# kerry-he/fsae-mpc

Hardware: AMD Instinct MI355X
Metric: QP solves/sec (batched LTV-MPC, N=40 nx=5 nu=2 fp64) (higher is better)
Workload: dtype f64

## Files before the change

### fsae-mpc_amd/csrc/qp_solver.hip

```cpp
#include <hip/hip_runtime.h>
#include <math.h>
#include <stdint.h>
#include <stdlib.h>
#include <stdio.h>
#include "qp_solver.h"

typedef double v4d __attribute__((ext_vector_type(4)));
typedef double v2d __attribute__((ext_vector_type(2)));

#define DEVINL __device__ __forceinline__
#ifndef QP_SOLVE_REFINE_STEPS
#define QP_SOLVE_REFINE_STEPS 1
#endif
#ifndef QP_FULL_BARRIERS
#define WAVE_SYNC() do { __builtin_amdgcn_fence(__ATOMIC_SEQ_CST, "wavefront"); __builtin_amdgcn_wave_barrier(); } while (0)
#else
#define WAVE_SYNC() __syncthreads()
#endif

namespace {

DEVINL double rl(double v, int src) {
  int lo = __builtin_amdgcn_readlane(__double2loint(v), src);
  int hi = __builtin_amdgcn_readlane(__double2hiint(v), src);
// ... 47 lines not shown
  __host__ __device__ static constexpr int idx(int I, int J) { return I * T - (I * (I - 1)) / 2 + (J - I); }
};

#if !defined(QP_TU) || QP_TU == 0
#define QP_MAIN_TU 1
#else
#define QP_MAIN_TU 0
#endif

#if QP_MAIN_TU
__global__ __launch_bounds__(1024) void qp_prep_kernel(QpParams P) {
  const int b = blockIdx.x, tid = threadIdx.x, w = tid >> 6, lane = tid & 63, c = lane & 15, q = lane >> 4;
  const int NTH = blockDim.x, NW = NTH >> 6;
  const QpDims& d = P.d;
  const int n = d.n, nu = d.nu, m = d.m, T = d.T, Kq = d.Kq, J = d.J, JB = d.JB, np = d.np, nc = d.nc, nb = d.nb;
  const double* H = P.H + (P.shared_HA ? 0 : (size_t)b * nu * nu);
  const double* A = P.A + (P.shared_HA ? 0 : (size_t)b * m * nu);
  const double* g = P.g + (size_t)b * nu;
  auto U = [&](int i) { return qp_user_index(d, i); };
  auto Hat = [&](int i, int j) -> double { const int ui = U(i), uj = U(j); return (ui >= 0 && uj >= 0) ? H[(size_t)uj * nu + ui] : ((i == j && i < n) ? 1.0 : 0.0); };
  auto Aat = [&](int r, int j) -> double { const int uj = U(j); return uj >= 0 ? A[(size_t)uj * m + r] : 0.0; };
  double* ws = P.ws + (size_t)b * d.ws_per_qp;
  double* Aw = ws + d.off_Aw;
  double* Hw = ws + d.off_Hw;
  double* gw = ws + d.off_gw;
  double* Es = ws + d.off_E;
  double* Fs = ws + d.off_F;
  double* Ab = ws + d.off_Ab;
  double* Hb = ws + d.off_Hb;
  int* perm_g = reinterpret_cast<int*>(ws + d.off_meta);
  int* tcs_g = perm_g + (size_t)(J > 0 ? J : 1) * 64;
  int* aoff_g = tcs_g + d.ntr;
  int* tend_g = aoff_g + d.ntr + 1;
  const int ntr = d.ntr;
  double* Lr = ws + d.off_rows + 0 * (size_t)d.rowlen;
  double* Ur = ws + d.off_rows + 1 * (size_t)d.rowlen;
  extern __shared__ double lds[];
  double* Esh = lds;
  double* red = lds + np;
  double* tile = red + 16;
  const int TW = d.prep_tw;
  int* cls_sh = reinterpret_cast<int*>(tile + TW * (4 * Kq + 1));
  int* perm_sh = cls_sh + 4 * Kq;
  int* cnt_sh = perm_sh + 16 * ntr;
  int* tcs_sh = cnt_sh + 16;
  int* aoff_sh = tcs_sh + ntr;
  int* chc_sh = aoff_sh + ntr + 1;
  double* Fr_sh = reinterpret_cast<double*>((reinterpret_cast<uintptr_t>(chc_sh + ((m + 63) >> 6) * 16) + 7) & ~(uintptr_t)7);

  for (int j = tid; j < np; j += NTH) {
    double e = 1.0;
    if (j < n) {
      double hjj = Hat(j, j);
      if (hjj > 1e-12) e = 1.0 / sqrt(hjj);
      else e = -1.0;
    } else e = 0.0;
    Esh[j] = e;
  }
  __syncthreads();
  for (int j = 0; j < n; ++j) {
    if (Esh[j] < 0) {
      double cm = 0;
      for (int r = tid; r < m; r += NTH) cm = fmax(cm, fabs(Aat(r, j)));
      cm = wave_max(cm);
      if (lane == 0) red[w] = cm;
      __syncthreads();
      if (tid == 0) { double mx = 0.0; for (int i = 0; i < NW; ++i) mx = fmax(mx, red[i]); Esh[j] = mx > 1e-12 ? 1.0 / mx : 1.0; }
      __syncthreads();
    }
  }
  int bad = 0;
  for (int j = tid; j < np; j += NTH) { const int uj = j < n ? U(j) : -1; const double gj = uj >= 0 ? g[uj] : 0.0; Es[j] = Esh[j]; gw[j] = gj * Esh[j]; bad |= !(fabs(gj) < INFINITY); }

  __syncthreads();
  const int ncols = nc < n ? nc : n;
  const int nchunk = (m + 63) >> 6;
  for (int i = tid; i < nchunk * 16; i += NTH) chc_sh[i] = 0;
  if (tid < 16) cnt_sh[tid] = 0;
  __syncthreads();
  for (int r0 = 0; r0 < m; r0 += NTH) {
    const int r = r0 + tid;
    int e = 0;
    double rm = 0.0;
    if (r < m) {
      for (int col0 = 0; col0 < n; col0 += 8) {
        double av[8];
#pragma unroll
        for (int u = 0; u < 8; ++u) av[u] = col0 + u < n ? Aat(r, col0 + u) : 0.0;
#pragma unroll
        for (int u = 0; u < 8; ++u) {
          const int col = col0 + u;
          const double a = fabs(av[u]);
          if (col < n) { rm = fmax(rm, a * Esh[col]); if (a != 0.0 && col < ncols) e = col >> 4; }
        }
      }
      cls_sh[r] = e;
      Fr_sh[r] = rm > 1e-12 ? 1.0 / rm : 1.0;
    }
    for (int cl = 0; cl < T; ++cl) {
      const unsigned long long mk = __ballot(r < m && e == cl);
      if (lane == 0 && r0 + 64 * w < m) chc_sh[((r0 >> 6) + w) * 16 + cl] = __popcll(mk);
    }
  }
  __syncthreads();
  if (tid < T) {
    int tot = 0;
    for (int ch = 0; ch < nchunk; ++ch) tot += chc_sh[ch * 16 + tid];
    cnt_sh[tid] = tot;
  }
  __syncthreads();
  if (tid < T) {
    int start = 0;
    for (int cl = 0; cl < tid; ++cl) start += cnt_sh[cl];
    for (int ch = 0; ch < nchunk; ++ch) { const int cn = chc_sh[ch * 16 + tid]; chc_sh[ch * 16 + tid] = start; start += cn; }
  }
  for (int p = tid; p < 16 * ntr; p += NTH) perm_sh[p] = -1;
  __syncthreads();
  for (int r0 = 0; r0 < m; r0 += NTH) {
    const int r = r0 + tid;
    const int e = r < m ? cls_sh[r] : -1;
    for (int cl = 0; cl < T; ++cl) {
      const unsigned long long mk = __ballot(e == cl);
      if (e == cl) perm_sh[chc_sh[((r0 >> 6) + w) * 16 + cl] + __popcll(mk & ((1ull << lane) - 1ull))] = r;
    }
  }
  __syncthreads();
  for (int tr = tid; tr < ntr; tr += NTH) {
    int tc = 1;
    for (int p = 16 * tr; p < 16 * tr + 16; ++p) { const int r = perm_sh[p]; if (r >= 0) tc = max(tc, cls_sh[r] + 1); }
    tcs_sh[tr] = tc;
  }
  __syncthreads();
  if (tid == 0) {
    int run = 0;
    for (int tr = 0; tr < ntr; ++tr) { aoff_sh[tr] = run; run += 2 * tcs_sh[tr]; }
    aoff_sh[ntr] = run;
    for (int C = 0; C <= T; ++C) { int cn = 0; for (int tr = 0; tr < ntr; ++tr) cn += (tcs_sh[tr] <= C); tend_g[C] = cn; }
  }
  __syncthreads();
  for (int tr = tid; tr <= ntr; tr += NTH) { aoff_g[tr] = aoff_sh[tr]; if (tr < ntr) tcs_g[tr] = tcs_sh[tr]; }

  int nexcl = 0;
  for (int js = w; js < J; js += NW) {
    const int s = 16 * js + c, pp = 4 * s + q;
    const int r = (s < 4 * ntr) ? perm_sh[pp] : -1;
    const bool valid = r >= 0;
    const double f = valid ? Fr_sh[r] : 0.0;
    Fs[js * 64 + lane] = f;
    perm_g[js * 64 + lane] = r;
    for (int bb = 0; bb < 4; ++bb)
    { const double v = (valid && bb < nb) ? Aat(r, nc + bb) * Esh[nc + bb] * f : 0.0; bad |= !(fabs(v) < INFINITY); Ab[(size_t)bb * J * 64 + js * 64 + lane] = v; }
    double l = -INFINITY, u = INFINITY;
    if (valid) {
      double lr = P.lbA[(size_t)b * m + r], ur = P.ubA[(size_t)b * m + r];
      bad |= (lr != lr) || (ur != ur);
      nexcl += (lr > 0.0) || (ur < 0.0);
      l = lr > -P.inf_bound ? lr * f : -INFINITY;
      u = ur < P.inf_bound ? ur * f : INFINITY;
    }
    Lr[js * 64 + lane] = l;
    Ur[js * 64 + lane] = u;
  }
  for (int jb = w; jb < JB; jb += NW) {
    const int i = jb * 64 + lane;
    double l = -INFINITY, u = INFINITY;
    const int ui = i < n ? U(i) : -1;
    if (ui >= 0) {
      double lr = P.lb[(size_t)b * nu + ui], ur = P.ub[(size_t)b * nu + ui];
      bad |= (lr != lr) || (ur != ur);
      nexcl += (lr > 0.0) || (ur < 0.0);
      l = lr > -P.inf_bound ? lr / Esh[i] : -INFINITY;
      u = ur < P.inf_bound ? ur / Esh[i] : INFINITY;
    }
    Lr[(J + jb) * 64 + lane] = l;
    Ur[(J + jb) * 64 + lane] = u;
  }
  __syncthreads();

  const int R4 = 4 * Kq, mp1 = R4 + 1;
  for (int t = 0; t < T; ++t)
    for (int c0 = 0; c0 < 16; c0 += TW) {
      for (int e = tid; e < TW * R4; e += NTH) {
        const int cc = e / R4, r = e - cc * R4;
        const int col = 16 * t + c0 + cc;
        double v = 0.0;
        if (col < nc && col < n && r < m) v = Aat(r, col) * Esh[col];
        bad |= !(fabs(v) < INFINITY);
        tile[cc * mp1 + r] = v;
      }
      __syncthreads();
      for (int s = w; s < 4 * ntr; s += NW) {
        const int tr = s >> 2, tc = tcs_sh[tr];
        if (t < tc && c >= c0 && c < c0 + TW) {
          const int r = perm_sh[4 * s + q];
          const double v = r >= 0 ? tile[(c - c0) * mp1 + r] * Fr_sh[r] : 0.0;
          Aw[((size_t)aoff_sh[tr] + ((s >> 1) & 1) * tc + t) * 128 + lane * 2 + (s & 1)] = v;
        }
      }
      __syncthreads();
    }

  for (int idx = w; idx < T * T * 4; idx += NW) {
    const int p = idx & 3, IJ = idx >> 2, I = IJ / T, Jt = IJ - I * T;
    const int row = 16 * I + q + 4 * p, col = 16 * Jt + c;
    double v = 0.0;
    if (row < nc && col < nc && row < n && col < n) v = Hat(col, row) * Esh[row] * Esh[col];
    bad |= !(fabs(v) < INFINITY);
    Hw[(size_t)idx * 64 + lane] = v;
  }
  for (int e = tid; e < 4 * np; e += NTH) {
    const int bb = e / np, i = e - bb * np;
    const double v = (bb < nb && i < n) ? Hat(i, nc + bb) * Esh[nc + bb] * Esh[i] : 0.0;
    bad |= !(fabs(v) < INFINITY);
    Hb[e] = v;
  }
  bad = __syncthreads_or(bad);
  if (tid == 0) ws[d.off_bad] = bad ? 1.0 : 0.0;
  if (P.score) {
    __shared__ int score_sh;
    if (tid == 0) score_sh = 0;
    __syncthreads();
    if (nexcl) atomicAdd(&score_sh, nexcl);
    __syncthreads();
    if (tid == 0) P.score[b] = P.score_in ? P.score_in[b] : score_sh;
  }
}

__global__ __launch_bounds__(1024) void qp_order_kernel(const int* __restrict__ score, int* __restrict__ order, int batch) {
  constexpr int NBIN = 1024, NWV = 8;
  __shared__ int cnt[NWV][NBIN], scan[NBIN];
  const int tid = threadIdx.x, w = tid >> 6, lane = tid & 63;
  for (int e = tid; e < NWV * NBIN; e += 1024) (&cnt[0][0])[e] = 0;
  __syncthreads();
  const int per = ((batch + NWV - 1) / NWV + 63) & ~63;
  const int lo = w * per, hi = min(batch, lo + per);
  auto bin = [&](int i) { return NBIN - 1 - min(max(score[i], 0), NBIN - 1); };
  auto group = [&](int k, bool on, int& rank, int& size) {
    unsigned long long same = __builtin_amdgcn_ballot_w64(on);
#pragma unroll
    for (int bit = 0; bit < 10; ++bit) {
      const bool one = (k >> bit) & 1;
      const unsigned long long v = __builtin_amdgcn_ballot_w64(one);
      same &= one ? v : ~v;
    }
    rank = __popcll(same & ((1ull << lane) - 1ull)); size = __popcll(same);
  };
  if (w < NWV)
    for (int i0 = lo; i0 < hi; i0 += 512) {
      int kv[8];
#pragma unroll
      for (int r = 0; r < 8; ++r) { const int i = i0 + 64 * r + lane; kv[r] = i < hi ? bin(i) : -1; }
#pragma unroll
      for (int r = 0; r < 8; ++r) {
        const bool on = kv[r] >= 0; const int k = on ? kv[r] : 0;
        int rank, size; group(k, on, rank, size);
        if (on && rank == 0) cnt[w][k] += size;
      }
    }
  __syncthreads();
  int v = 0;
  for (int ww = 0; ww < NWV; ++ww) v += cnt[ww][tid];
  scan[tid] = v;
  __syncthreads();
  for (int o = 1; o < NBIN; o <<= 1) {
    const int a = tid >= o ? scan[tid - o] : 0;
    __syncthreads();
    scan[tid] += a;
    __syncthreads();
  }
  int run = scan[tid] - v;
  for (int ww = 0; ww < NWV; ++ww) { const int c = cnt[ww][tid]; cnt[ww][tid] = run; run += c; }
  __syncthreads();
  if (w < NWV)
    for (int i0 = lo; i0 < hi; i0 += 512) {
      int kv[8];
#pragma unroll
      for (int r = 0; r < 8; ++r) { const int i = i0 + 64 * r + lane; kv[r] = i < hi ? bin(i) : -1; }
#pragma unroll
      for (int r = 0; r < 8; ++r) {
        const bool on = kv[r] >= 0; const int k = on ? kv[r] : 0;
        int rank, size; group(k, on, rank, size);
        int base = on ? cnt[w][k] : 0;
        if (on) order[base + rank] = i0 + 64 * r + lane;
        if (on && rank == 0) cnt[w][k] = base + size;
      }
    }
}

#endif

struct Ctx {
  int n, m, T, Kq, J, JB, JT, np, ld, lane, c, q, nc, nb, ntr;
  const int* perm; const int* tcs; const int* aoff; const int* tend;
  const double* Aw; const double* Hw; const double* Ab; const double* Hb;
  double* rows;
  double* ring;
  double* cof;
  int rowlen;
  double* Ms;
  double* vec;
};
enum VecArr { V_X = 0, V_G, V_HX, V_R1, V_R2, V_P1, V_P2, V_P3, V_DX, V_E, V_NARR };

DEVINL double* rowp(const Ctx& k, int arr) { return k.rows + (size_t)arr * k.rowlen; }
DEVINL double* vecp(const Ctx& k, int arr) { return k.vec + arr * k.np; }

DEVINL bool row_valid(const Ctx& k, int js) {
  if (js < k.J) { const int s = 16 * js + k.c; return s < k.Kq && 4 * s + k.q < k.m; }
  return (js - k.J) * 64 + k.lane < k.n;
}

template <int T> DEVINL void hx_tiles(const Ctx& k, const double* X, double* HX) {
  double hx[T], hn[T][4], hc[T][4];
#pragma unroll
  for (int t = 0; t < T; ++t) hx[t] = 0.0;
#pragma unroll
  for (int Jt = 0; Jt < T; ++Jt)
#pragma unroll
    for (int p = 0; p < 4; ++p) hn[Jt][p] = k.Hw[((size_t)Jt * 4 + p) * 64 + k.lane];
#pragma unroll 1
  for (int I = 0; I < T; ++I) {
#pragma unroll
    for (int Jt = 0; Jt < T; ++Jt)
#pragma unroll
      for (int p = 0; p < 4; ++p) hc[Jt][p] = hn[Jt][p];
    if (I + 1 < T) {
#pragma unroll
      for (int Jt = 0; Jt < T; ++Jt)
#pragma unroll
        for (int p = 0; p < 4; ++p) hn[Jt][p] = k.Hw[((size_t)((I + 1) * T + Jt) * 4 + p) * 64 + k.lane];
    }
    double xk[4];
#pragma unroll
    for (int p = 0; p < 4; ++p) xk[p] = X[16 * I + k.q + 4 * p];
#pragma unroll
    for (int Jt = 0; Jt < T; ++Jt)
#pragma unroll
      for (int p = 0; p < 4; ++p) hx[Jt] = fma(hc[Jt][p], xk[p], hx[Jt]);
  }
#pragma unroll
  for (int t = 0; t < T; ++t) {
    double v = q_sum(hx[t]);
    if (k.q == 0) HX[16 * t + k.c] = v;
  }
}
template <int T> DEVINL void acc_init(const Ctx& k, v4d* acc) {
#pragma unroll
  for (int I = 0; I < T; ++I)
#pragma unroll
    for (int Jt = I; Jt < T; ++Jt) {
      const double* hp = k.Hw + ((size_t)(I * T + Jt) * 4) * 64 + k.lane;
      v4d h;
#pragma unroll
      for (int p = 0; p < 4; ++p) h[p] = hp[p * 64];
      acc[Tri<T>::idx(I, Jt)] = h;
    }
}

template <int T> DEVINL void hx_from_acc(const Ctx& k, const v4d* acc, const double* XV, double* HX) {
  double xr[T][4], xc[T], sc[T], sr[T][4];
#pragma unroll
  for (int I = 0; I < T; ++I) {
    xc[I] = XV[16 * I + k.c]; sc[I] = 0.0;
#pragma unroll
    for (int p = 0; p < 4; ++p) { xr[I][p] = XV[16 * I + k.q + 4 * p]; sr[I][p] = 0.0; }
  }
#pragma unroll
  for (int I = 0; I < T; ++I)
#pragma unroll
    for (int J = I; J < T; ++J) {
      const v4d& h = acc[Tri<T>::idx(I, J)];
#pragma unroll
      for (int p = 0; p < 4; ++p) {
        sc[J] = fma(h[p], xr[I][p], sc[J]);
        if (J > I) sr[I][p] = fma(h[p], xc[J], sr[I][p]);
      }
    }
  WAVE_SYNC();
#pragma unroll
  for (int J = 0; J < T; ++J) { const double v = q_sum(sc[J]); if (k.q == 0) HX[16 * J + k.c] = v; }
  WAVE_SYNC();
#pragma unroll
  for (int I = 0; I < T - 1; ++I)
#pragma unroll
    for (int p = 0; p < 4; ++p) { const double v = grp16_sum(sr[I][p]); if (k.c == 0) HX[16 * I + k.q + 4 * p] += v; }
}

template <int C> struct IC { static constexpr int value = C; };

#ifdef QP_DRAIN_STREAM
template <int T> struct StreamCfg {
  static constexpr int R = 3 * T;
};
template <int T> struct Stream {
  static constexpr int R = StreamCfg<T>::R;
  const char* gnext;
  int half;
  DEVINL void issue(const Ctx& k, int slot) {
    __builtin_amdgcn_global_load_lds((const __attribute__((address_space(1))) void*)(gnext + k.lane * 16),
                                     (__attribute__((address_space(3))) void*)(k.ring + slot * 128), 16, 0, 0);
    gnext += 1024;
  }
  DEVINL void start(const Ctx& k, int c0) {
    gnext = reinterpret_cast<const char*>(k.Aw); half = 0;
#pragma unroll
    for (int t = 0; t < T; ++t) if (t < c0) issue(k, t);
  }
  template <int C> DEVINL void next_pair(const Ctx& k, v2d* b, int cn) {
    asm volatile("s_waitcnt vmcnt(0)" ::: "memory");
    const int other = (half ^ 1) * T;
#pragma unroll
    for (int t = 0; t < T; ++t) if (t < cn) issue(k, other + t);
    asm volatile("" ::: "memory");
#pragma unroll
    for (int t = 0; t < C; ++t) b[t] = *reinterpret_cast<const v2d*>(k.ring + (half * T + t) * 128 + k.lane * 2);
    half ^= 1;
  }
  DEVINL void drain() { asm volatile("s_waitcnt vmcnt(0)" ::: "memory"); }
};
#else
template <int T> struct StreamCfg {
  static constexpr int D = 2 * T;
  static constexpr int R = D + T;
};
template <int T> struct Stream {
  static constexpr int D = StreamCfg<T>::D, R = StreamCfg<T>::R;
  const char* gnext; int slot_i, slot_e;
  DEVINL void issue(const Ctx& k) {
    __builtin_amdgcn_global_load_lds((const __attribute__((address_space(1))) void*)(gnext + k.lane * 16),
                                     (__attribute__((address_space(3))) void*)(k.ring + slot_i * 128), 16, 0, 0);
    gnext += 1024;
    slot_i = slot_i + 1 == R ? 0 : slot_i + 1;
  }
  DEVINL void start(const Ctx& k, int) {
    gnext = reinterpret_cast<const char*>(k.Aw); slot_i = 0; slot_e = 0;
#pragma unroll
    for (int j = 0; j < D; ++j) issue(k);
  }
  template <int C> DEVINL void next_pair(const Ctx& k, v2d* b, int) {
#pragma unroll
    for (int t = 0; t < C; ++t) issue(k);
    asm volatile("s_waitcnt vmcnt(%0)" :: "n"(D) : "memory");
#pragma unroll
    for (int t = 0; t < C; ++t) {
      int sl = slot_e + t; if (sl >= R) sl -= R;
      b[t] = *reinterpret_cast<const v2d*>(k.ring + sl * 128 + k.lane * 2);
    }
    slot_e += C; if (slot_e >= R) slot_e -= R;
  }
  DEVINL void drain() { asm volatile("s_waitcnt vmcnt(0)" ::: "memory"); }
};
#endif

template <int NA> struct CoefStage {
  double reg[NA > 0 ? NA : 1];
  DEVINL void load(const Ctx& k, const double* const* arr, int js) {
    const int jc = js < k.J ? js : k.J - 1;
#pragma unroll
    for (int a = 0; a < NA; ++a) reg[a] = arr[a][jc * 64 + k.lane];
  }
  DEVINL void commit(const Ctx& k) {
#pragma unroll
    for (int a = 0; a < NA; ++a) k.cof[a * 64 + k.lane] = reg[a];
  }
  DEVINL void read_pair(const Ctx& k, int s, v2d* out) const {
#pragma unroll
    for (int a = 0; a < NA; ++a) out[a] = *reinterpret_cast<const v2d*>(k.cof + a * 64 + k.q * 16 + (s & 15));
  }
};

template <int T, int NB> DEVINL void pass_syrk(const Ctx& k, v4d* acc, double* P1, double* P2, double* P3, double* MB) {
  constexpr int NBB = NB > 0 ? NB : 1;
  constexpr int NA = 4 + NB;
  const int JS = k.J * 64;
  const double* arr[NA];
  arr[0] = rowp(k, R_D); arr[1] = rowp(k, R_W1); arr[2] = rowp(k, R_W2); arr[3] = rowp(k, R_W3);
#pragma unroll
  for (int e = 0; e < NB; ++e) arr[4 + e] = k.Ab + (size_t)e * JS;
  double p1[T], p2[T], p3[T];
  double pb[NBB][T], sbb[NBB][NBB], pwb[3][NBB];
#pragma unroll
  for (int t = 0; t < T; ++t) { p1[t] = 0; p2[t] = 0; p3[t] = 0; }
#pragma unroll
  for (int e = 0; e < NBB; ++e) {
#pragma unroll
    for (int t = 0; t < T; ++t) pb[e][t] = 0;
#pragma unroll
    for (int f = 0; f < NBB; ++f) sbb[e][f] = 0;
    pwb[0][e] = pwb[1][e] = pwb[2][e] = 0;
  }
  Stream<T> st;
  CoefStage<NA> cs;
  int tr = 0;
  if (k.ntr > 0) { st.start(k, k.tcs[0]); cs.load(k, arr, 0); }
  auto phase = [&](auto Cc) __attribute__((always_inline)) {
    constexpr int C = decltype(Cc)::value;
    const int tr_end = k.tend[C];
    for (; tr < tr_end; ++tr) {
      if ((tr & 3) == 0) { cs.commit(k); cs.load(k, arr, (tr >> 2) + 1); }
#pragma unroll
      for (int u = 0; u < 2; ++u) {
        v2d b[C], cf[NA];
        st.template next_pair<C>(k, b, u == 0 ? C : (tr + 1 < tr_end ? C : (tr + 1 < k.ntr ? k.tcs[tr + 1] : 0)));
        cs.read_pair(k, 4 * tr + 2 * u, cf);
        asm volatile("" ::: "memory");
#pragma unroll
        for (int h = 0; h < 2; ++h) {
          double a[C], ab[NBB];
          const double dd = cf[0][h], w1 = cf[1][h], w2 = cf[2][h], w3 = cf[3][h];
#pragma unroll
          for (int e = 0; e < NB; ++e) ab[e] = cf[4 + e][h];
#pragma unroll
          for (int t = 0; t < C; ++t) a[t] = dd * b[t][h];
#pragma unroll
          for (int I = 0; I < C; ++I)
#pragma unroll
            for (int Jt = I; Jt < C; ++Jt)
              acc[Tri<T>::idx(I, Jt)] = __builtin_amdgcn_mfma_f64_16x16x4f64(a[I], b[Jt][h], acc[Tri<T>::idx(I, Jt)], 0, 0, 0);
#pragma unroll
          for (int t = 0; t < C; ++t) {
            p1[t] = fma(w1, b[t][h], p1[t]); p2[t] = fma(w2, b[t][h], p2[t]); p3[t] = fma(w3, b[t][h], p3[t]);
          }
#pragma unroll
          for (int e = 0; e < NB; ++e) {
            const double dab = dd * ab[e];
#pragma unroll
            for (int t = 0; t < C; ++t) pb[e][t] = fma(dab, b[t][h], pb[e][t]);
#pragma unroll
            for (int f = e; f < NB; ++f) sbb[e][f] = fma(dab, ab[f], sbb[e][f]);
            pwb[0][e] = fma(w1, ab[e], pwb[0][e]); pwb[1][e] = fma(w2, ab[e], pwb[1][e]); pwb[2][e] = fma(w3, ab[e], pwb[2][e]);
          }
        }
      }
    }
  };
  if constexpr (T >= 1) phase(IC<1>{});
  if constexpr (T >= 2) phase(IC<2>{});
  if constexpr (T >= 3) phase(IC<3>{});
  if constexpr (T >= 4) phase(IC<4>{});
  if constexpr (T >= 5) phase(IC<5>{});
  if constexpr (T >= 6) phase(IC<6>{});
  if constexpr (T >= 7) phase(IC<7>{});
  if constexpr (T >= 8) phase(IC<8>{});
  if (k.ntr > 0) st.drain();
#pragma unroll
  for (int t = 0; t < T; ++t) {
    double v1 = q_sum(p1[t]), v2 = q_sum(p2[t]), v3 = q_sum(p3[t]);
    if (k.q == 0) { P1[16 * t + k.c] = v1; P2[16 * t + k.c] = v2; P3[16 * t + k.c] = v3; }
  }
#pragma unroll
  for (int e = 0; e < NB; ++e) {
#pragma unroll
    for (int t = 0; t < T; ++t) { const double vb = q_sum(pb[e][t]); if (k.q == 0) MB[e * k.np + 16 * t + k.c] = vb; }
    const double v1 = q_sum(pwb[0][e]), v2 = q_sum(pwb[1][e]), v3 = q_sum(pwb[2][e]);
    if (k.lane == 0) { P1[k.nc + e] = v1; P2[k.nc + e] = v2; P3[k.nc + e] = v3; }
#pragma unroll
    for (int f = 0; f < NB; ++f) {
      const double sv = q_sum(f >= e ? sbb[e][f] : sbb[f][e]);
      if (k.lane == 0) MB[e * k.np + k.nc + f] = sv;
    }
  }
}

template <int T, int NB, int NVEC, int FUSE> DEVINL void pass_Av(const Ctx& k, const double* const* vin, double* const* rout, double* Pcor, double* Pcor2 = nullptr, const double* const* cfarr = nullptr) {
  constexpr int NBB = NB > 0 ? NB : 1;
  constexpr int NC = FUSE == 1 ? 6 : (FUSE >= 2 ? 3 : 0);
  constexpr int NA = NC + NB;
  const int JS = k.J * 64;
  const double* arr[NA > 0 ? NA : 1];
  if (FUSE == 1) { arr[0] = rowp(k, R_RPL); arr[1] = rowp(k, R_CB1); arr[2] = rowp(k, R_CC1); arr[3] = rowp(k, R_RPU); arr[4] = rowp(k, R_CB2); arr[5] = rowp(k, R_CC2); }
  if (FUSE >= 2) { arr[0] = cfarr ? cfarr[0] : rowp(k, R_CB1); arr[1] = cfarr ? cfarr[1] : rowp(k, R_RPL); arr[2] = cfarr ? cfarr[2] : rowp(k, R_CC1); }
#pragma unroll
  for (int f = 0; f < NB; ++f) arr[NC + f] = k.Ab + (size_t)f * JS;
  double v[NVEC][T], vb[NVEC][NBB], pc[T], pcb[NBB], pd[FUSE >= 2 ? T : 1], pdb[NBB];
#pragma unroll
  for (int e = 0; e < NVEC; ++e) {
#pragma unroll
    for (int t = 0; t < T; ++t) v[e][t] = vin[e][16 * t + k.c];
#pragma unroll
    for (int f = 0; f < NB; ++f) vb[e][f] = vin[e][k.nc + f];
  }
#pragma unroll
  for (int t = 0; t < T; ++t) pc[t] = 0.0;
#pragma unroll
  for (int f = 0; f < NBB; ++f) { pcb[f] = 0.0; pdb[f] = 0.0; }
#pragma unroll
  for (int t = 0; t < (FUSE >= 2 ? T : 1); ++t) pd[t] = 0.0;
  double keep[NVEC + 1];
#pragma unroll
  for (int e = 0; e < NVEC + 1; ++e) keep[e] = 0.0;
  Stream<T> st;
  CoefStage<NA> cs;
  int tr = 0;
  if (k.ntr > 0) { st.start(k, k.tcs[0]); if (NA > 0) cs.load(k, arr, 0); }
  auto phase = [&](auto Cc) __attribute__((always_inline)) {
    constexpr int C = decltype(Cc)::value;
    const int tr_end = k.tend[C];
    for (; tr < tr_end; ++tr) {
      if (NA > 0 && (tr & 3) == 0) { cs.commit(k); cs.load(k, arr, (tr >> 2) + 1); }
#pragma unroll
      for (int u = 0; u < 2; ++u) {
        v2d b[C], cf[NA > 0 ? NA : 1];
        st.template next_pair<C>(k, b, u == 0 ? C : (tr + 1 < tr_end ? C : (tr + 1 < k.ntr ? k.tcs[tr + 1] : 0)));
        if (NA > 0) cs.read_pair(k, 4 * tr + 2 * u, cf);
        asm volatile("" ::: "memory");
#pragma unroll
        for (int h = 0; h < 2; ++h) {
          const int s = 4 * tr + 2 * u + h;
          const int cc = s & 15;
#pragma unroll
          for (int e = 0; e < NVEC; ++e) {
            double dsum = 0.0;
#pragma unroll
            for (int t = 0; t < C; ++t) dsum = fma(b[t][h], v[e][t], dsum);
            dsum = grp16_sum(dsum);
#pragma unroll
            for (int f = 0; f < NB; ++f) dsum = fma(cf[NC + f][h], vb[e][f], dsum);
            if (k.c == cc) keep[e] = dsum;
            if (FUSE >= 2 && e == 0) {
              const double pen = cf[0][h] * (dsum - cf[1][h]);
              const double ynew = cf[2][h] - pen;
              if (k.c == cc) keep[NVEC] = ynew;
#pragma unroll
              for (int t = 0; t < C; ++t) { pc[t] = fma(ynew, b[t][h], pc[t]); pd[t] = fma(pen, b[t][h], pd[t]); }
#pragma unroll
              for (int f = 0; f < NB; ++f) { pcb[f] = fma(ynew, cf[NC + f][h], pcb[f]); pdb[f] = fma(pen, cf[NC + f][h], pdb[f]); }
            }
            if (FUSE == 1 && e == 0) {
              const double dl_ = dsum + cf[0][h], du_ = cf[3][h] - dsum;
              const double w = dl_ * fma(cf[2][h], dl_, cf[1][h]) - du_ * fma(cf[5][h], du_, cf[4][h]);
#pragma unroll
              for (int t = 0; t < C; ++t) pc[t] = fma(w, b[t][h], pc[t]);
#pragma unroll
              for (int f = 0; f < NB; ++f) pcb[f] = fma(w, cf[NC + f][h], pcb[f]);
            }
          }
          if (cc == 15 || s + 1 == 4 * k.ntr) {
            const int js = s >> 4;
#pragma unroll
            for (int e = 0; e < NVEC; ++e) { rout[e][js * 64 + k.lane] = keep[e]; keep[e] = 0.0; }
            if (FUSE >= 2) { rout[NVEC][js * 64 + k.lane] = keep[NVEC]; keep[NVEC] = 0.0; }
          }
        }
      }
    }
  };
  if constexpr (T >= 1) phase(IC<1>{});
  if constexpr (T >= 2) phase(IC<2>{});
  if constexpr (T >= 3) phase(IC<3>{});
  if constexpr (T >= 4) phase(IC<4>{});
  if constexpr (T >= 5) phase(IC<5>{});
  if constexpr (T >= 6) phase(IC<6>{});
  if constexpr (T >= 7) phase(IC<7>{});
  if constexpr (T >= 8) phase(IC<8>{});
  if (k.ntr > 0) st.drain();
  if (FUSE) {
#pragma unroll
    for (int t = 0; t < T; ++t) {
      double pv = q_sum(pc[t]);
      if (k.q == 0) Pcor[16 * t + k.c] = pv;
    }
#pragma unroll
    for (int f = 0; f < NB; ++f) { const double pv = q_sum(pcb[f]); if (k.lane == 0) Pcor[k.nc + f] = pv; }
  }
  if (FUSE >= 2) {
#pragma unroll
    for (int t = 0; t < T; ++t) {
      double pv = q_sum(pd[t]);
      if (k.q == 0) Pcor2[16 * t + k.c] = pv;
    }
#pragma unroll
    for (int f = 0; f < NB; ++f) { const double pv = q_sum(pdb[f]); if (k.lane == 0) Pcor2[k.nc + f] = pv; }
  }
}

template <int T, int NB> DEVINL void pass_Atw(const Ctx& k, const double* W, double* Pout) {
  constexpr int NBB = NB > 0 ? NB : 1;
  const int JS = k.J * 64;
  double p[T], pbv[NBB];
#pragma unroll
  for (int t = 0; t < T; ++t) p[t] = 0.0;
#pragma unroll
  for (int f = 0; f < NBB; ++f) pbv[f] = 0.0;
  for (int s = 0; s < 4 * k.ntr; ++s) {
    const int ri = (s >> 4) * 64 + k.q * 16 + (s & 15);
    const double w = W[ri];
    const int tr = s >> 2, tc = k.tcs[tr];
    const double* src = k.Aw + ((size_t)k.aoff[tr] + ((s >> 1) & 1) * tc) * 128 + k.lane * 2 + (s & 1);
#pragma unroll
    for (int t = 0; t < T; ++t)
      if (t < tc) p[t] = fma(w, src[t * 128], p[t]);
#pragma unroll
    for (int f = 0; f < NB; ++f) pbv[f] = fma(w, k.Ab[(size_t)f * JS + ri], pbv[f]);
  }
#pragma unroll
  for (int t = 0; t < T; ++t) {
    double v = q_sum(p[t]);
    if (k.q == 0) Pout[16 * t + k.c] = v;
  }
#pragma unroll
  for (int f = 0; f < NB; ++f) { const double pv = q_sum(pbv[f]); if (k.lane == 0) Pout[k.nc + f] = pv; }
}

template <int T> DEVINL void mfma4_sub(const v4d& X, const v4d& Y, v4d& Dst) {
#pragma unroll
  for (int p = 0; p < 4; ++p) Dst = __builtin_amdgcn_mfma_f64_16x16x4f64(-X[p], Y[p], Dst, 0, 0, 0);
}
DEVINL v4d mfma4_new(const v4d& X, const v4d& Y) {
  v4d Z = {0.0, 0.0, 0.0, 0.0};
#pragma unroll
  for (int p = 0; p < 4; ++p) Z = __builtin_amdgcn_mfma_f64_16x16x4f64(X[p], Y[p], Z, 0, 0, 0);
  return Z;
}

DEVINL v4d tile_transpose(const Ctx& k, double* scratch, const v4d& Xt) {
  WAVE_SYNC();
#pragma unroll
  for (int p = 0; p < 4; ++p) scratch[(k.q + 4 * p) * 17 + k.c] = Xt[p];
  WAVE_SYNC();
  v4d Z;
#pragma unroll
  for (int p = 0; p < 4; ++p) Z[p] = scratch[k.c * 17 + k.q + 4 * p];
  return Z;
}

DEVINL void tile_store(const Ctx& k, double* slot, const v4d& Xt) {
#pragma unroll
  for (int p = 0; p < 4; ++p) slot[(k.q + 4 * p) * 17 + k.c] = Xt[p];
}
DEVINL v4d tile_load(const Ctx& k, const double* slot) {
  v4d Z;
#pragma unroll
  for (int p = 0; p < 4; ++p) Z[p] = slot[(k.q + 4 * p) * 17 + k.c];
  return Z;
}
DEVINL v4d tile_load_t(const Ctx& k, const double* slot) {
  v4d Z;
#pragma unroll
  for (int p = 0; p < 4; ++p) Z[p] = slot[k.c * 17 + k.q + 4 * p];
  return Z;
}

DEVINL int diag_factor(const Ctx& k, v4d& Ud, v4d& Yk, v4d& rk, double floor_abs) {
  int bad = 0;
#pragma unroll
  for (int p = 0; p < 4; ++p) {
    const double d00 = rl(Ud[p], 4 * p + 0), d01 = rl(Ud[p], 4 * p + 1), d02 = rl(Ud[p], 4 * p + 2), d03 = rl(Ud[p], 4 * p + 3);
    const double d11 = rl(Ud[p], 16 + 4 * p + 1), d12 = rl(Ud[p], 16 + 4 * p + 2), d13 = rl(Ud[p], 16 + 4 * p + 3);
    const double d22 = rl(Ud[p], 32 + 4 * p + 2), d23 = rl(Ud[p], 32 + 4 * p + 3);
    const double d33 = rl(Ud[p], 48 + 4 * p + 3);
    auto piv = [&](double t) { if (!(t > floor_abs)) { if (!(fabs(t) < INFINITY)) bad = 1; t = floor_abs; } return rsqrt(t); };
    const double i0 = piv(d00);
    const double r01 = d01 * i0, r02 = d02 * i0, r03 = d03 * i0;
    const double i1 = piv(fma(-r01, r01, d11));
    const double r12 = fma(-r01, r02, d12) * i1, r13 = fma(-r01, r03, d13) * i1;
    const double i2 = piv(fma(-r12, r12, fma(-r02, r02, d22)));
    const double r23 = fma(-r12, r13, fma(-r02, r03, d23)) * i2;
    const double i3 = piv(fma(-r23, r23, fma(-r13, r13, fma(-r03, r03, d33))));
    const double w10 = -r01 * i0 * i1;
    const double w20 = -fma(r12, w10, r02 * i0) * i2, w21 = -r12 * i1 * i2;
    const double w30 = -fma(r23, w20, fma(r13, w10, r03 * i0)) * i3, w31 = -fma(r23, w21, r13 * i1) * i3, w32 = -r23 * i2 * i3;
    const int a_ = k.c - 4 * p;
    double wa = 0.0;
    if (k.q == 0) wa = a_ == 0 ? i0 : (a_ == 1 ? w10 : (a_ == 2 ? w20 : (a_ == 3 ? w30 : 0.0)));
    if (k.q == 1) wa = a_ == 1 ? i1 : (a_ == 2 ? w21 : (a_ == 3 ? w31 : 0.0));
    if (k.q == 2) wa = a_ == 2 ? i2 : (a_ == 3 ? w32 : 0.0);
    if (k.q == 3) wa = a_ == 3 ? i3 : 0.0;
    const v4d z = {0.0, 0.0, 0.0, 0.0};
    const v4d nu = __builtin_amdgcn_mfma_f64_16x16x4f64(wa, Ud[p], z, 0, 0, 0);
    const v4d ny = __builtin_amdgcn_mfma_f64_16x16x4f64(wa, Yk[p], z, 0, 0, 0);
    const v4d nr = __builtin_amdgcn_mfma_f64_16x16x4f64(wa, rk[p], z, 0, 0, 0);
    Ud[p] = nu[p]; Yk[p] = ny[p]; rk[p] = nr[p];
    if (p < 3) {
      const double a = (k.c > 4 * p + 3) ? -Ud[p] : 0.0;
      Yk = __builtin_amdgcn_mfma_f64_16x16x4f64(a, Yk[p], Yk, 0, 0, 0);
      rk = __builtin_amdgcn_mfma_f64_16x16x4f64(a, rk[p], rk, 0, 0, 0);
      Ud = __builtin_amdgcn_mfma_f64_16x16x4f64(a, Ud[p], Ud, 0, 0, 0);
    }
  }
#pragma unroll
  for (int p = 0; p < 4; ++p) if (k.c < k.q + 4 * p) Ud[p] = 0.0;
  return bad;
}

template <int T, int K, bool RHS> struct FactorStep {
  static DEVINL int run(const Ctx& k, v4d* acc, double* YL, v4d* rh, double floor_abs) {
    v4d Yk, none = {0.0, 0.0, 0.0, 0.0};
#pragma unroll
    for (int p = 0; p < 4; ++p) Yk[p] = (k.q + 4 * p == k.c) ? 1.0 : 0.0;
    int bad = diag_factor(k, acc[Tri<T>::idx(K, K)], Yk, RHS ? rh[K] : none, floor_abs);
    tile_store(k, YL + K * 272, Yk);
    WAVE_SYNC();
    const v4d Wk = tile_load_t(k, YL + K * 272);
    const v4d& UKK = acc[Tri<T>::idx(K, K)];
#pragma unroll
    for (int Jt = K + 1; Jt < T; ++Jt) {
      v4d Rr = acc[Tri<T>::idx(K, Jt)];
      v4d Ukj = mfma4_new(Wk, Rr);
#ifndef QP_NO_ROW_REFINE
      mfma4_sub<T>(UKK, Ukj, Rr);
#pragma unroll
      for (int p = 0; p < 4; ++p) Ukj = __builtin_amdgcn_mfma_f64_16x16x4f64(Wk[p], Rr[p], Ukj, 0, 0, 0);
#endif
      acc[Tri<T>::idx(K, Jt)] = Ukj;
    }
#pragma unroll
    for (int I = K + 1; I < T; ++I) {
      const v4d& UKI = acc[Tri<T>::idx(K, I)];
#pragma unroll
      for (int Jt = I; Jt < T; ++Jt) mfma4_sub<T>(UKI, acc[Tri<T>::idx(K, Jt)], acc[Tri<T>::idx(I, Jt)]);
      if (RHS) mfma4_sub<T>(UKI, rh[K], rh[I]);
    }
    return bad | FactorStep<T, K + 1, RHS>::run(k, acc, YL, rh, floor_abs);
  }
};
template <int T, bool RHS> struct FactorStep<T, T, RHS> {
  static DEVINL int run(const Ctx&, v4d*, double*, v4d*, double) { return 0; }
};
template <int T> DEVINL int reg_factor(const Ctx& k, v4d* acc, double* YL, v4d* rh, double floor_abs) {
  return FactorStep<T, 0, true>::run(k, acc, YL, rh, floor_abs);
}
template <int T> DEVINL int reg_factor_only(const Ctx& k, v4d* acc, double* YL, double floor_abs) {
  return FactorStep<T, 0, false>::run(k, acc, YL, nullptr, floor_abs);
}

template <int T> DEVINL void reg_forward(const Ctx& k, const v4d* acc, const double* YL, v4d* rh) {
#pragma unroll
  for (int K = 0; K < T; ++K) {
    rh[K] = mfma4_new(tile_load_t(k, YL + K * 272), rh[K]);
#pragma unroll
    for (int I = K + 1; I < T; ++I) mfma4_sub<T>(acc[Tri<T>::idx(K, I)], rh[K], rh[I]);
  }
}

template <int T> DEVINL void reg_backward(const Ctx& k, const v4d* acc, const double* YL, v4d* rh, double* scratch) {
#pragma unroll
  for (int K = T - 1; K >= 0; --K) {
#pragma unroll
    for (int Jt = K + 1; Jt < T; ++Jt) {
      const v4d Lt = tile_transpose(k, scratch, acc[Tri<T>::idx(K, Jt)]);
      mfma4_sub<T>(Lt, rh[Jt], rh[K]);
    }
    rh[K] = mfma4_new(tile_load(k, YL + K * 272), rh[K]);
  }
}

template <int T, bool REFINE> DEVINL void vec_forward(const Ctx& k, const v4d* acc, const double* YL, const double* B, double (&y)[T][4]) {
#pragma unroll
  for (int K = 0; K < T; ++K) {
    double s = 0.0;
#pragma unroll
    for (int I = 0; I < K; ++I)
#pragma unroll
      for (int p = 0; p < 4; ++p) s = fma(acc[Tri<T>::idx(I, K)][p], y[I][p], s);
    const double t = B[16 * K + k.c] - (K > 0 ? q_sum(s) : 0.0);
    const v4d Yt = tile_load(k, YL + K * 272);
#pragma unroll
    for (int p = 0; p < 4; ++p) y[K][p] = grp16_sum(Yt[p] * t);
    if (REFINE) {
      const v4d& U = acc[Tri<T>::idx(K, K)];
#pragma unroll
      for (int rep = 0; rep < QP_SOLVE_REFINE_STEPS; ++rep) {
        double r = 0.0;
#pragma unroll
        for (int p = 0; p < 4; ++p) r = fma(U[p], y[K][p], r);
        r = t - q_sum(r);
#pragma unroll
        for (int p = 0; p < 4; ++p) y[K][p] += grp16_sum(Yt[p] * r);
      }
    }
  }
}
template <int T, bool REFINE> DEVINL void vec_backward(const Ctx& k, const v4d* acc, const double* YL, const double (&y)[T][4], double* X) {
  double x[T];
#pragma unroll
  for (int K = T - 1; K >= 0; --K) {
    const v4d Yt = tile_load(k, YL + K * 272);
    double w[4], s2 = 0.0;
#pragma unroll
    for (int p = 0; p < 4; ++p) {
      double s = 0.0;
#pragma unroll
      for (int J = K + 1; J < T; ++J) s = fma(acc[Tri<T>::idx(K, J)][p], x[J], s);
      w[p] = y[K][p] - (K < T - 1 ? grp16_sum(s) : 0.0);
      s2 = fma(Yt[p], w[p], s2);
    }
    x[K] = q_sum(s2);
    if (REFINE) {
      const v4d& U = acc[Tri<T>::idx(K, K)];
#pragma unroll
      for (int rep = 0; rep < QP_SOLVE_REFINE_STEPS; ++rep) {
        double d = 0.0;
#pragma unroll
        for (int p = 0; p < 4; ++p) d = fma(Yt[p], w[p] - grp16_sum(U[p] * x[K]), d);
        x[K] += q_sum(d);
      }
    }
    if (k.q == 0) X[16 * K + k.c] = x[K];
  }
}
template <int T> DEVINL void vec_rows_store(const Ctx& k, const double (&y)[T][4], double* V) {
  if (k.c == 0) {
#pragma unroll
    for (int K = 0; K < T; ++K)
#pragma unroll
      for (int p = 0; p < 4; ++p) V[16 * K + k.q + 4 * p] = y[K][p];
// ... 1343 lines not shown
```

Measured before the change: 376,600.

## Stream coefficient tiles via direct global-to-LDS loads with double-buffered half-slabs

```diff
diff --git a/fsae-mpc_amd/csrc/qp_solver.hip b/fsae-mpc_amd/csrc/qp_solver.hip
--- a/fsae-mpc_amd/csrc/qp_solver.hip
+++ b/fsae-mpc_amd/csrc/qp_solver.hip
@@ -373,6 +373,8 @@
 };
 enum VecArr { V_X = 0, V_G, V_HX, V_R1, V_R2, V_P1, V_P2, V_P3, V_DX, V_E, V_NARR };
 
+DEVINL int dir_load(const int* p) { return *(const __attribute__((address_space(4))) int*)p; }
+
 DEVINL double* rowp(const Ctx& k, int arr) { return k.rows + (size_t)arr * k.rowlen; }
 DEVINL double* vecp(const Ctx& k, int arr) { return k.vec + arr * k.np; }
 
@@ -461,6 +463,7 @@
 
 #ifdef QP_DRAIN_STREAM
 template <int T> struct StreamCfg {
+  static constexpr int D = 0;
   static constexpr int R = 3 * T;
 };
 template <int T> struct Stream {
@@ -487,7 +490,7 @@
     for (int t = 0; t < C; ++t) b[t] = *reinterpret_cast<const v2d*>(k.ring + (half * T + t) * 128 + k.lane * 2);
     half ^= 1;
   }
-  DEVINL void drain() { asm volatile("s_waitcnt vmcnt(0)" ::: "memory"); }
+  DEVINL void drain() { asm volatile("s_waitcnt vmcnt(0) ; stream drain" ::: "memory"); }
 };
 #else
 template <int T> struct StreamCfg {
@@ -519,24 +522,28 @@
     }
     slot_e += C; if (slot_e >= R) slot_e -= R;
   }
-  DEVINL void drain() { asm volatile("s_waitcnt vmcnt(0)" ::: "memory"); }
+  DEVINL void drain() { asm volatile("s_waitcnt vmcnt(0) ; stream drain" ::: "memory"); }
 };
 #endif
 
 template <int NA> struct CoefStage {
-  double reg[NA > 0 ? NA : 1];
-  DEVINL void load(const Ctx& k, const double* const* arr, int js) {
-    const int jc = js < k.J ? js : k.J - 1;
-#pragma unroll
-    for (int a = 0; a < NA; ++a) reg[a] = arr[a][jc * 64 + k.lane];
-  }
-  DEVINL void commit(const Ctx& k) {
-#pragma unroll
-    for (int a = 0; a < NA; ++a) k.cof[a * 64 + k.lane] = reg[a];
+  static constexpr int HS = NA * 32;
+  DEVINL void issue(const Ctx& k, const double* const* arr, int hs) {
+    const int js = hs >> 1, jc = js < k.J ? js : k.J - 1;
+    const int off = (jc * 64 + k.q * 16 + (hs & 1) * 8) * 8 + k.c * 4;
+    double* dst = k.cof + (hs & 1) * HS;
+#pragma unroll
+    for (int a = 0; a < NA; ++a)
+      __builtin_amdgcn_global_load_lds((const __attribute__((address_space(1))) void*)(reinterpret_cast<const char*>(arr[a]) + off),
+                                       (__attribute__((address_space(3))) void*)(dst + a * 32), 4, 0, 0);
+  }
+  template <int C, int D> DEVINL void first_pair_wait() const {
+    if constexpr (4 + C + NA < D) asm volatile("s_waitcnt vmcnt(%0)" :: "n"(4 + C + NA) : "memory");
   }
   DEVINL void read_pair(const Ctx& k, int s, v2d* out) const {
-#pragma unroll
-    for (int a = 0; a < NA; ++a) out[a] = *reinterpret_cast<const v2d*>(k.cof + a * 64 + k.q * 16 + (s & 15));
+    const double* base = k.cof + ((s >> 3) & 1) * HS + k.q * 8 + (s & 7);
+#pragma unroll
+    for (int a = 0; a < NA; ++a) out[a] = *reinterpret_cast<const v2d*>(base + a * 32);
   }
 };
 
@@ -563,16 +570,18 @@
   Stream<T> st;
   CoefStage<NA> cs;
   int tr = 0;
-  if (k.ntr > 0) { st.start(k, k.tcs[0]); cs.load(k, arr, 0); }
+  asm volatile("s_waitcnt vmcnt(0)" ::: "memory");
+  if (k.ntr > 0) { cs.issue(k, arr, 0); st.start(k, dir_load(k.tcs)); }
   auto phase = [&](auto Cc) __attribute__((always_inline)) {
     constexpr int C = decltype(Cc)::value;
-    const int tr_end = k.tend[C];
+    const int tr_end = dir_load(k.tend + C);
     for (; tr < tr_end; ++tr) {
-      if ((tr & 3) == 0) { cs.commit(k); cs.load(k, arr, (tr >> 2) + 1); }
+      if ((tr & 1) == 0) cs.issue(k, arr, (tr >> 1) + 1);
 #pragma unroll
       for (int u = 0; u < 2; ++u) {
         v2d b[C], cf[NA];
-        st.template next_pair<C>(k, b, u == 0 ? C : (tr + 1 < tr_end ? C : (tr + 1 < k.ntr ? k.tcs[tr + 1] : 0)));
+        st.template next_pair<C>(k, b, u == 0 ? C : (tr + 1 < tr_end ? C : (tr + 1 < k.ntr ? dir_load(k.tcs + tr + 1) : 0)));
+        if (u == 0 && (tr & 1) == 0) cs.template first_pair_wait<C, StreamCfg<T>::D>();
         cs.read_pair(k, 4 * tr + 2 * u, cf);
         asm volatile("" ::: "memory");
 #pragma unroll
@@ -663,16 +672,18 @@
   Stream<T> st;
   CoefStage<NA> cs;
   int tr = 0;
-  if (k.ntr > 0) { st.start(k, k.tcs[0]); if (NA > 0) cs.load(k, arr, 0); }
+  asm volatile("s_waitcnt vmcnt(0)" ::: "memory");
+  if (k.ntr > 0) { if (NA > 0) cs.issue(k, arr, 0); st.start(k, dir_load(k.tcs)); }
   auto phase = [&](auto Cc) __attribute__((always_inline)) {
     constexpr int C = decltype(Cc)::value;
-    const int tr_end = k.tend[C];
+    const int tr_end = dir_load(k.tend + C);
     for (; tr < tr_end; ++tr) {
-      if (NA > 0 && (tr & 3) == 0) { cs.commit(k); cs.load(k, arr, (tr >> 2) + 1); }
+      if (NA > 0 && (tr & 1) == 0) cs.issue(k, arr, (tr >> 1) + 1);
 #pragma unroll
       for (int u = 0; u < 2; ++u) {
         v2d b[C], cf[NA > 0 ? NA : 1];
-        st.template next_pair<C>(k, b, u == 0 ? C : (tr + 1 < tr_end ? C : (tr + 1 < k.ntr ? k.tcs[tr + 1] : 0)));
+        st.template next_pair<C>(k, b, u == 0 ? C : (tr + 1 < tr_end ? C : (tr + 1 < k.ntr ? dir_load(k.tcs + tr + 1) : 0)));
+        if (NA > 0 && u == 0 && (tr & 1) == 0) cs.template first_pair_wait<C, StreamCfg<T>::D>();
         if (NA > 0) cs.read_pair(k, 4 * tr + 2 * u, cf);
         asm volatile("" ::: "memory");
 #pragma unroll
```

Result: no change. 375,500, median of 6 (-0.3%).
